# HorizonRobotics/GeoFlowSlam

Hardware: AMD Instinct MI355X
Metric: front-end frames/sec (ORB+match+GICP) on 640x480 RGBD (higher is better)
Workload: dtype u8/int32 (ORB, match) + f64 (GICP); 1 GPU; BASELINE.json configs[1]: 640x480 RGBD frame pair, ORB extract (1000 feats, 8 levels) + BF Hamming match + GMS filter + GICP on ~19k-pt clouds (stride-4 depth grid); batch_pairs_per_gpu=512, lanes_per_gpu=4, passes=K passes per lane chain, joined once, distinct_scenes_per_gpu=512, scene_seeds=1000..1511 (rank 0), global_batch_pairs=512, parallelism=frames sharded x1, no collective

## Files before the change

geoflowslam_amd/csrc/gicp.hip:

```cpp
#include <algorithm>
#include <atomic>
#include <cmath>
#include <cstdlib>
#include <memory>
#include <type_traits>

#include "gfs_common.hpp"
#include "glibc_math.hpp"
#include "voxel_qsort.hpp"
#include "wave_reduce.hpp"

namespace {

typedef unsigned long long u64;
constexpr u64 kInvalidKey = ~0ull;
constexpr int kCoordBits = 21;
constexpr int kCoordOffset = 1 << (kCoordBits - 1);
constexpr int kCoordMask = (1 << kCoordBits) - 1;
#ifndef GFS_FINE_BITS
#define GFS_FINE_BITS 6
#endif
constexpr int kFineBits = GFS_FINE_BITS, kFine = 1 << kFineBits;
static_assert(kFineBits >= 1 && kFineBits <= 6, "the x field of a cell sort key: 19 bits of cell + the sub-cell bits in 25");
constexpr int kCkSy = 25, kCkSz = 45;
constexpr int kCkOffX = 1 << 24, kCkOffY = 1 << 19, kCkOffZ = 1 << 18;
constexpr int kRed = 29;
constexpr int kLinBlock = 256;

struct PairState {
  double T[12];
  double newT[12];
  double delta[6];
  double H[21], b[6], e;
  double lambda;
  int outer, inner;
  int phase;
  int converged;
  int iterations;
  int inliers;
  int n_lin, n_err;
  int buf;
  int pad_;
};

struct GicpParams {
  double inv_leaf, cell, inv_cell, max_dist_sq, rot_eps, trans_eps;
  int max_iterations, k_neighbors;
  unsigned* tile_stats;
  int lin_tile;
  int nn_rings;
  int src_slot, only;
  int knn_exact;
};

__device__ __forceinline__ int fast_floor_d(double v) {
  const int n = (int)v;
  return n - (v < (double)n ? 1 : 0);
}
__device__ __forceinline__ u64 pack_key(int cx, int cy, int cz) {
  return (u64)(cx & kCoordMask) | ((u64)(cy & kCoordMask) << kCoordBits) | ((u64)(cz & kCoordMask) << (2 * kCoordBits));
}

__global__ __launch_bounds__(256) void k_voxel_keys(const float4* __restrict__ tgt, const float4* __restrict__ src,
                                                    const int* __restrict__ nt, const int* __restrict__ ns,
                                                    int stride_pts, int P, double inv_leaf, double max_vox, u64* __restrict__ keys,
                                                    unsigned* __restrict__ idx, int* __restrict__ counts, int only,
                                                    int* __restrict__ n_done4, int* __restrict__ n_heap, int* __restrict__ n_active4) {
  const int c = blockIdx.y, pair = c >> 1, which = c & 1;
  if (blockIdx.x == 0 && threadIdx.x < 4) {
    if (threadIdx.x == 0) n_heap[c] = 0;
    if (c == 0) {
      n_done4[threadIdx.x] = 0;
      n_active4[threadIdx.x] = 0;
    }
  }
  if (only >= 0 && which != only) return;
  const int n = min(which ? ns[pair] : nt[pair], P);
  const float4* in = (which ? src : tgt) + (size_t)pair * stride_pts;
  const int i = blockIdx.x * 256 + threadIdx.x;
  if (i == 0) counts[c] = n;
  if (i >= n) return;
  const float4 p = in[i];
  const double x = (double)p.x * inv_leaf, y = (double)p.y * inv_leaf, z = (double)p.z * inv_leaf;
  u64 key = kInvalidKey;
  if (fabs(x) < max_vox && fabs(y) < max_vox && fabs(z) < max_vox) {
    const int cx = fast_floor_d(x) + kCoordOffset, cy = fast_floor_d(y) + kCoordOffset, cz = fast_floor_d(z) + kCoordOffset;
// ... 987 lines not shown
    atomicAdd(util + slot, (unsigned)__popcll(m));
    atomicAdd(util + slot + 1, 1u);
  }
}
#define GFS_KNN_UTIL_STEP(util, slot) knn_util_step(util, slot)
#else
#define GFS_KNN_UTIL_STEP(util, slot)
#endif
__device__ __forceinline__ void knn_walk_own_row(const double4* __restrict__ p, const double4& q, int i, int lo, int hi, double slack,
                                                 int want, TopKey11& loc, unsigned* util = nullptr) {
  int r = i, l = i - 1;
  bool ra = r < hi, la = l >= lo;
  const int kw_at = max(want - 1, 0);
  while (ra || la) {
    GFS_KNN_UTIL_STEP(util, 0);
    const int j0 = min(r, hi - 1), j1 = max(l, lo), j2 = min(r + 1, hi - 1), j3 = max(l - 1, lo);
    const bool on2 = ra && r + 1 < hi, on3 = la && l - 1 >= lo;
    const double4 t0 = ld_pt(p, j0), t1 = ld_pt(p, j1), t2 = ld_pt(p, j2), t3 = ld_pt(p, j3);
    loc.push4(knn_key(t0, q, j0, ra), knn_key(t1, q, j1, la), knn_key(t2, q, j2, on2), knn_key(t3, q, j3, on3));
    const double kw = loc.at(kw_at);
    const double B = kw < TopKey11::kNone ? TopKey11::upper(kw) : TopKey11::kNone;
    if (ra) {
      r += 2;
      const double g = t2.x - slack - q.x;
      ra = r < hi && !(g > 0.0 && g * g > B);
    }
    if (la) {
      l -= 2;
      const double g = q.x - t3.x - slack;
      la = l >= lo && !(g > 0.0 && g * g > B);
    }
  }
}
__device__ __forceinline__ void knn_scan_runs4_keys(const double4* __restrict__ p, const double4& q, int b0, int l0, int b1, int l1,
                                                    int b2, int l2, int b3, int l3, TopKey11& loc, unsigned* util = nullptr) {
  const int c1 = l0, c2 = c1 + l1, c3 = c2 + l2, total = c3 + l3;
  const int o0 = b0, o1 = b1 - c1, o2 = b2 - c2, o3 = b3 - c3;
  for (int v = 0; v < total; v += 4) {
    GFS_KNN_UTIL_STEP(util, 2);
    int j[4];
#pragma unroll
    for (int u = 0; u < 4; u++) {
      const int vv = min(v + u, total - 1);
      j[u] = vv + (vv < c1 ? o0 : vv < c2 ? o1 : vv < c3 ? o2 : o3);
    }
    const int j0 = j[0], j1 = j[1], j2 = j[2], j3 = j[3];
    const double4 t0 = ld_pt(p, j0), t1 = ld_pt(p, j1), t2 = ld_pt(p, j2), t3 = ld_pt(p, j3);
    loc.push4(knn_key(t0, q, j0, true), knn_key(t1, q, j1, v + 1 < total), knn_key(t2, q, j2, v + 2 < total),
              knn_key(t3, q, j3, v + 3 < total));
  }
}

__device__ __forceinline__ void knn_write_cov(const TopK<10>& best, int kk, const double4* __restrict__ p, double* __restrict__ out) {
  const int n = min(best.found, kk);
  if (n < 5) {
    out[0] = 1;
    out[1] = 0;
    out[2] = 0;
    out[3] = 1;
    out[4] = 0;
    out[5] = 1;
    return;
  }
  double sp[3] = {0, 0, 0}, sc[6] = {0, 0, 0, 0, 0, 0};
#pragma unroll
  for (int k = 0; k < 10; k++) {
    if (k < n) {
      const double4 t = p[best.id[k]];
      sp[0] += t.x;
      sp[1] += t.y;
      sp[2] += t.z;
      sc[0] += t.x * t.x;
      sc[1] += t.x * t.y;
      sc[2] += t.x * t.z;
      sc[3] += t.y * t.y;
      sc[4] += t.y * t.z;
      sc[5] += t.z * t.z;
    }
  }
  const double dn = (double)n;
  const double mean[3] = {sp[0] / dn, sp[1] / dn, sp[2] / dn};
  double cv[6];
  cv[0] = (sc[0] - mean[0] * sp[0]) / dn;
  cv[1] = (sc[1] - mean[1] * sp[0]) / dn;
// ... 37 lines not shown
}

__device__ __forceinline__ void knn_scan_runs4(const double4* __restrict__ p, const double4& q, int b0, int l0, int b1, int l1, int b2,
                                               int l2, int b3, int l3, TopK<10>& loc) {
  const int c1 = l0, c2 = c1 + l1, c3 = c2 + l2, total = c3 + l3;
  const int o0 = b0, o1 = b1 - c1, o2 = b2 - c2, o3 = b3 - c3;
  for (int v = 0; v < total; v += 4) {
    int j[4];
#pragma unroll
    for (int u = 0; u < 4; u++) {
      const int vv = min(v + u, total - 1);
      j[u] = vv + (vv < c1 ? o0 : vv < c2 ? o1 : vv < c3 ? o2 : o3);
    }
    const double4 t0 = p[j[0]], t1 = p[j[1]], t2 = p[j[2]], t3 = p[j[3]];
    {
      const double ddx = t0.x - q.x, ddy = t0.y - q.y, ddz = t0.z - q.z;
      loc.push(j[0], ddx * ddx + ddy * ddy + ddz * ddz);
    }
    if (v + 1 < total) {
      const double ddx = t1.x - q.x, ddy = t1.y - q.y, ddz = t1.z - q.z;
      loc.push(j[1], ddx * ddx + ddy * ddy + ddz * ddz);
    }
    if (v + 2 < total) {
      const double ddx = t2.x - q.x, ddy = t2.y - q.y, ddz = t2.z - q.z;
      loc.push(j[2], ddx * ddx + ddy * ddy + ddz * ddz);
    }
    if (v + 3 < total) {
      const double ddx = t3.x - q.x, ddy = t3.y - q.y, ddz = t3.z - q.z;
      loc.push(j[3], ddx * ddx + ddy * ddy + ddz * ddz);
    }
  }
}

__global__ __launch_bounds__(128) void k_knn_cov(const double4* __restrict__ pts, const u64* __restrict__ ucell,
                                                 const unsigned* __restrict__ ubegin, const int* __restrict__ n_ucell,
                                                 const int* __restrict__ m_counts, const int* __restrict__ bbox,
                                                 const unsigned* __restrict__ grid, const int* __restrict__ ginfo,
                                                 int* __restrict__ ginfo_rw, unsigned* __restrict__ hard_list,
                                                 double* __restrict__ hard_d, int nchunks, int npairs, int P, GicpParams prm,
                                                 double* __restrict__ cov6) {
  int pair, which, chunk;
  if (!xcd_pair_map(nchunks, npairs, 2, &pair, &which, &chunk)) return;
  if (prm.only >= 0 && which != prm.only) return;
  const int c = 2 * pair + which;
  const int m = m_counts[c];
  const int i = chunk * 128 + threadIdx.x;
  if (i >= m) return;
  const unsigned* G = grid + (size_t)c * (kGridCap + 1);
  const int* gi = ginfo + 8 * c;
  const double4* p = pts + (size_t)c * P;
  const u64* uc = ucell + (size_t)c * (P + 1);
  const unsigned* ub = ubegin + (size_t)c * (P + 1);
  const int nu = n_ucell[c];
  const double4 q = p[i];
  const int cx = fast_floor_d(q.x * prm.inv_cell) + kCoordOffset, cy = fast_floor_d(q.y * prm.inv_cell) + kCoordOffset,
            cz = fast_floor_d(q.z * prm.inv_cell) + kCoordOffset;
  TopKey11 best;
  const int kk = min(prm.k_neighbors, 10);
  const int want = min(kk, m);
  bool certified = false;
  double kth_for_deferred = TopKey11::kNone;
  {
    best.init();
    const double cell2 = prm.cell * prm.cell;
    const double ux = q.x * prm.inv_cell - (double)(cx - kCoordOffset), uy = q.y * prm.inv_cell - (double)(cy - kCoordOffset),
                 uz = q.z * prm.inv_cell - (double)(cz - kCoordOffset);
    const double lx0 = fmax(ux - 1e-9, 0.0) * prm.cell, lx2 = fmax(1.0 - ux - 1e-9, 0.0) * prm.cell;
    const double ly[3] = {fmax(uy - 1e-9, 0.0) * prm.cell, 0.0, fmax(1.0 - uy - 1e-9, 0.0) * prm.cell};
    const double lz[3] = {fmax(uz - 1e-9, 0.0) * prm.cell, 0.0, fmax(1.0 - uz - 1e-9, 0.0) * prm.cell};
    {
      int j0, j1;
      row_range(gi, G, uc, ub, nu, cx - 1, cx + 1, cy, cz, &j0, &j1);
#ifdef GFS_KNN_OWN_ROW_SCAN
      knn_scan_run_keys(p, q, j0, j1, best);
#else
      if (i >= j0 && i < j1)
        knn_walk_own_row(p, q, i, j0, j1, prm.cell * (1.0 / kFine + 1e-9), want, best, prm.tile_stats);
      else
        knn_scan_run_keys(p, q, j0, j1, best);
#endif
    }
    auto kth_bound = [&]() {
      const double kw = best.at(max(want - 1, 0));
      return kw < TopKey11::kNone ? TopKey11::upper(kw) : TopKey11::kNone;
    };
    constexpr int rows[2][4] = {{1, 3, 5, 7}, {0, 2, 6, 8}};
#pragma unroll
    for (int round = 0; round < 2; round++) {
      const double B = kth_bound();
      int rb[4], rl[4];
#pragma unroll
      for (int u = 0; u < 4; u++) {
        const int t9 = rows[round][u], dy = t9 % 3, dz = t9 / 3;
        const double row2 = ly[dy] * ly[dy] + lz[dz] * lz[dz];
        rb[u] = 0;
        rl[u] = 0;
        if (row2 <= B) {
          int e[4];
          row_cells3(gi, G, uc, ub, nu, cx, cy + dy - 1, cz + dz - 1, e);
          const int b0 = row2 + lx0 * lx0 <= B ? e[0] : e[1], e0 = row2 + lx2 * lx2 <= B ? e[3] : e[2];
          rb[u] = b0;
          rl[u] = e0 - b0;
        }
      }
      knn_scan_runs4_keys(p, q, rb[0], rl[0], rb[1], rl[1], rb[2], rl[2], rb[3], rl[3], best, prm.tile_stats);
    }
#ifdef GFS_KNN_UTIL
    if (prm.tile_stats) {
      GFS_KNN_UTIL_STEP(prm.tile_stats, 4);
      int j0, j1;
      row_range(gi, G, uc, ub, nu, cx - 1, cx + 1, cy, cz, &j0, &j1);
      atomicAdd(prm.tile_stats + 6, (unsigned)(j1 - j0));
    }
#endif
    const double fx = fmin(ux + 1.0, 2.0 - ux), fy = fmin(uy + 1.0, 2.0 - uy), fz = fmin(uz + 1.0, 2.0 - uz);
    const double reach = fmax(fmin(fx, fmin(fy, fz)) - 1e-9, 1.0) * prm.cell;
    const double kw = best.at(max(want - 1, 0)), kn = best.at(want);
    certified = want > 0 && kw < TopKey11::kNone && TopKey11::upper(kw) <= fmax(reach * reach, cell2) &&
                !(kn < TopKey11::kNone && TopKey11::same_high_bits(kw, kn));
    certified = (certified || want == 0) && !prm.knn_exact;
    kth_for_deferred = kw < TopKey11::kNone ? TopKey11::upper(kw) : TopKey11::kNone;
  }
  if (!certified) {
    const int slot = atomicAdd(&ginfo_rw[8 * c + 7], 1);
    hard_list[(size_t)c * P + slot] = (unsigned)i;
    hard_d[(size_t)c * P + slot] = kth_for_deferred;
    return;
  }
  TopK<10> res;
  res.found = 0;
#pragma unroll
  for (int k = 0; k < 10; k++) {
    res.id[k] = best.k[k] < TopKey11::kNone ? TopKey11::index(best.k[k]) : -1;
    res.found += best.k[k] < TopKey11::kNone ? 1 : 0;
  }
  knn_write_cov(res, kk, p, cov6 + ((size_t)c * P + i) * 6);
}

// ... 545 lines not shown
      atomicAdd(src.util + 7, 1u);
    }
  }
#endif
  row(cy, cz, 0.0);
  unsigned need = 0;
#pragma unroll
  for (int t8 = 0; t8 < 8; t8++) {
    const int t9 = t8 < 4 ? t8 : t8 + 1, dy = t9 % 3, dz = t9 / 3;
    const double a = dy == 0 ? ly0 : dy == 2 ? ly2 : 0.0, c = dz == 0 ? lz0 : dz == 2 ? lz2 : 0.0;
    if (a * a + c * c <= B) need |= 1u << t8;
  }
  while (__any(need != 0)) {
#ifdef GFS_LIN_UTIL
    if (src.util) {
      const unsigned long long m = __ballot(need != 0);
      if ((int)(threadIdx.x & 63) == __ffsll((long long)__ballot(1)) - 1) {
        atomicAdd(src.util + 2, (unsigned)__popcll(m));
        atomicAdd(src.util + 3, 1u);
      }
    }
#endif
    if (need != 0) {
      const int t8 = __ffs(need) - 1;
      need &= need - 1;
      const int t9 = t8 < 4 ? t8 : t8 + 1, dy = t9 % 3, dz = t9 / 3;
      const double a = dy == 0 ? ly0 : dy == 2 ? ly2 : 0.0, c = dz == 0 ? lz0 : dz == 2 ? lz2 : 0.0;
      const double row2 = a * a + c * c;
      if (row2 <= B) row(cy + dy - 1, cz + dz - 1, row2);
    }
  }
}

__device__ __forceinline__ int lin_stage_tile(LinTile& T, bool inrange, int cx, int cy, int cz, const double4* __restrict__ tp,
                                              const int* __restrict__ gi, const unsigned* __restrict__ G) {
  const int tid = threadIdx.x, lane = tid & 63, wave = tid >> 6;
  if (!gi[6]) return 1;
  if (tid < 4) T.box[tid] = (tid & 1) ? INT_MIN : INT_MAX;
  if (tid < kTileRows) {
    T.row_a[tid] = INT_MAX;
    T.row_b[tid] = INT_MIN;
  }
  __syncthreads();
  {
    int v[4] = {inrange ? cy : INT_MAX, inrange ? -cy : INT_MAX, inrange ? cz : INT_MAX, inrange ? -cz : INT_MAX};
#pragma unroll
    for (int ofs = 32; ofs > 0; ofs >>= 1)
#pragma unroll
      for (int k = 0; k < 4; k++) v[k] = min(v[k], __shfl_xor(v[k], ofs, 64));
    if (lane == 0 && v[0] != INT_MAX) {
      atomicMin(&T.box[0], v[0]);
      atomicMax(&T.box[1], -v[1]);
      atomicMin(&T.box[2], v[2]);
      atomicMax(&T.box[3], -v[3]);
    }
  }
  __syncthreads();
  const int cymin = T.box[0], cymax = T.box[1], czmin = T.box[2], czmax = T.box[3];
  if (cymin > cymax) return 2;
  const long long nyl = (long long)cymax - cymin + 3, nzl = (long long)czmax - czmin + 3;
  if (nyl * nzl > kTileRows) return 3;
  const int ny = (int)nyl, nz = (int)nzl, nrows = ny * nz, y0 = cymin - 1, z0 = czmin - 1;
  if (inrange) {
    const int r = (cy - y0) + ny * (cz - z0);
    atomicMin(&T.row_a[r], cx);
    atomicMax(&T.row_b[r], cx);
// ... 189 lines not shown
  v[3] = fmsub2(F.Q[5], F.px, F.Q[3], F.pz);
  v[4] = fmsub2(F.Q[8], F.px, F.Q[6], F.pz);
  v[5] = fmsub2(F.Q[6], F.py, F.Q[7], F.px);
  v[6] = fmsub2(F.u[1], F.pz, F.u[2], F.py);
  v[7] = fmsub2(F.u[2], F.px, F.u[0], F.pz);
  v[8] = fmsub2(F.u[0], F.py, F.u[1], F.px);
  v[9] = -F.u[0];
  v[10] = -F.u[1];
  v[11] = -F.u[2];
  v[12] = 0.5 * fma3(F.w[0], F.u[0], F.w[1], F.u[1], F.w[2], F.u[2]);
  v[13] = 1.0;
}
__device__ __forceinline__ void lin_factor_batch_a(const LinFactor& F, double (&v)[15]) {
#pragma unroll
  for (int k = 0; k < 15; k++) v[k] = 0;
  if (!F.on) return;
#pragma unroll
  for (int c = 0; c < 3; c++)
#pragma unroll
    for (int r = 0; r < 3; r++) v[3 * c + r] = -F.Q[c + 3 * r];
#pragma unroll
  for (int k = 0; k < 6; k++) v[9 + k] = F.N[k];
}
__device__ __forceinline__ void lin_factor_accumulate(const LinFactor& F, double (&acc)[kRed]) {
  double a[15], b[14];
  lin_factor_batch_a(F, a);
  lin_factor_batch_b(F, b);
#pragma unroll
  for (int k = 0; k < 15; k++) acc[kLinMapA[k]] += a[k];
#pragma unroll
  for (int k = 0; k < 14; k++) acc[kLinMapB[k]] += b[k];
}

template <class Src>
__device__ __forceinline__ void gicp_lin_point(const Src& src, int i, const double4 p, double tx, double ty, double tz, int cx, int cy, int cz,
                                               bool in_range, const double* __restrict__ T12, bool has_prev, int prev_j, const double4 prev_q,
                                               int pair, int cs, int ct, int P,
                                               const double4* __restrict__ pts, const double* __restrict__ cov6,
                                               const u64* __restrict__ ucell, const unsigned* __restrict__ ubegin,
                                               const int* __restrict__ n_ucell, const unsigned* __restrict__ G,
                                               const int* __restrict__ gi, const GicpParams& prm, int* __restrict__ tgt_index,
                                               double* __restrict__ maha6, LinFactor& F) {
  {
    const double4* tp = pts + (size_t)ct * P;
    const u64* uc = ucell + (size_t)ct * (P + 1);
    const unsigned* ub = ubegin + (size_t)ct * (P + 1);
    const int nu = n_ucell[ct];
    double best = 1.79769313486231570e308;
    int bj = -1;
    if (in_range) {
      if (prm.nn_rings <= 1) {
        if (has_prev && prev_j >= 0) {
          best = (prev_q.x - tx) * (prev_q.x - tx) + (prev_q.y - ty) * (prev_q.y - ty) + (prev_q.z - tz) * (prev_q.z - tz);
          bj = prev_j;
        }
        nn_search27(src, prm, tx, ty, tz, cx, cy, cz, best, bj);
      } else {
      {
        int j0s[9], j1s[9];
#pragma unroll
        for (int t9 = 0; t9 < 9; t9++)
          row_range(gi, G, uc, ub, nu, cx - 1, cx + 1, cy + (t9 % 3) - 1, cz + t9 / 3 - 1, &j0s[t9], &j1s[t9]);
#pragma unroll
        for (int t9 = 0; t9 < 9; t9++) {
          const int jb = j0s[t9], je = j1s[t9];
          for (int j = jb; j < je; j += 4) {
            const int ja = min(j + 1, je - 1), jb2 = min(j + 2, je - 1), jc = min(j + 3, je - 1);
            const double4 q0 = tp[j], q1 = tp[ja], q2 = tp[jb2], q3 = tp[jc];
            const double d0 = (q0.x - tx) * (q0.x - tx) + (q0.y - ty) * (q0.y - ty) + (q0.z - tz) * (q0.z - tz);
            const double d1 = (q1.x - tx) * (q1.x - tx) + (q1.y - ty) * (q1.y - ty) + (q1.z - tz) * (q1.z - tz);
            const double d2 = (q2.x - tx) * (q2.x - tx) + (q2.y - ty) * (q2.y - ty) + (q2.z - tz) * (q2.z - tz);
            const double d3 = (q3.x - tx) * (q3.x - tx) + (q3.y - ty) * (q3.y - ty) + (q3.z - tz) * (q3.z - tz);
            if (d0 < best) { best = d0; bj = j; }
            if (d1 < best) { best = d1; bj = ja; }
            if (d2 < best) { best = d2; bj = jb2; }
            if (d3 < best) { best = d3; bj = jc; }
          }
        }
      }
      const bool done1 = (bj >= 0 && best <= prm.cell * prm.cell) || prm.nn_rings <= 1;
      for (int r = 2; !done1 && r <= prm.nn_rings; r++) {
        best = 1.79769313486231570e308;
        bj = -1;
        for (int dz = -r; dz <= r; dz++)
          for (int dy = -r; dy <= r; dy++) {
            int j0, j1;
            row_range(gi, G, uc, ub, nu, cx - r, cx + r, cy + dy, cz + dz, &j0, &j1);
            for (int j = j0; j < j1; j++) {
              const double4 q = tp[j];
// ... 19 lines not shown

__device__ __forceinline__ void lin_image(const double4& p, const double* __restrict__ T12, const GicpParams& prm, double& tx, double& ty,
                                          double& tz, int& cx, int& cy, int& cz, bool& in_range) {
  const double* R = T12;
  const double* t = T12 + 9;
  tx = R[0] * p.x + R[3] * p.y + R[6] * p.z + t[0];
  ty = R[1] * p.x + R[4] * p.y + R[7] * p.z + t[1];
  tz = R[2] * p.x + R[5] * p.y + R[8] * p.z + t[2];
  cx = fast_floor_d(tx * prm.inv_cell) + kCoordOffset;
  cy = fast_floor_d(ty * prm.inv_cell) + kCoordOffset;
  cz = fast_floor_d(tz * prm.inv_cell) + kCoordOffset;
  in_range = fabs(tx) < 2.0e4 && fabs(ty) < 2.0e4 && fabs(tz) < 2.0e4;
}

#ifdef GFS_LIN_WAVES
#define GFS_LIN_OCC __attribute__((amdgpu_waves_per_eu(GFS_LIN_WAVES, 8)))
#else
#define GFS_LIN_OCC __attribute__((amdgpu_waves_per_eu(5, 8)))
#endif
struct CoopSync {
  unsigned arrive;
  unsigned gen;
};
__device__ void pair_step_last(PairState* S, const double* part, const double* epart, int nblk_pair, int phase, double rot_eps,
                               double trans_eps, int max_iterations, int pair, int* n_done, int* act_next, int* n_act_next, double* s_part,
                               double* s_sum);

__device__ __forceinline__ double gicp_trial_error(const double4 q, double tx, double ty, double tz, const double* __restrict__ M) {
  const double r0 = q.x - tx, r1 = q.y - ty, r2 = q.z - tz;
  const double m0 = M[0] * r0 + M[1] * r1 + M[2] * r2, m1 = M[1] * r0 + M[3] * r1 + M[4] * r2, m2 = M[2] * r0 + M[4] * r1 + M[5] * r2;
  return 0.5 * (r0 * m0 + r1 * m1 + r2 * m2);
}

template <bool kTiled, bool kFuse>
__global__ __launch_bounds__(kLinBlock) GFS_LIN_OCC void k_gicp_linearize(PairState* __restrict__ st,
                                                              const double4* __restrict__ pts,
                                                              const double* __restrict__ cov6, const u64* __restrict__ ucell,
                                                              const unsigned* __restrict__ ubegin,
                                                              const int* __restrict__ n_ucell, const int* __restrict__ m_counts,
                                                              const unsigned* __restrict__ grid, const int* __restrict__ ginfo,
                                                              int nchunks, int npairs, int P, GicpParams prm,
                                                              int* __restrict__ tgt_index, double* __restrict__ maha6, size_t buf_stride,
                                                              double* __restrict__ partial, double* __restrict__ epartial, int nblk,
                                                              const int* __restrict__ act, const int* __restrict__ n_act,
                                                              CoopSync* __restrict__ sync, int* __restrict__ n_done,
                                                              int* __restrict__ act_next, int* __restrict__ n_act_next,
                                                              int* __restrict__ n_act_clear) {
  __shared__ typename std::conditional<kTiled, LinTile, int>::type tile;
  if constexpr (kFuse) {
    if (blockIdx.x == 0 && threadIdx.x == 0) *n_act_clear = 0;
  }
  int pair, sub, chunk;
  if (act) {
    const int slot = blockIdx.x / nchunks;
    if (slot >= *n_act) return;
    pair = act[slot];
    chunk = blockIdx.x - slot * nchunks;
  } else if (!xcd_pair_map(nchunks, npairs, 1, &pair, &sub, &chunk)) {
    return;
  }
  const int cs = 2 * pair + prm.src_slot, ct = 2 * pair + 1 - prm.src_slot;
  const PairState* Sp = st + pair;
  const int phase = Sp->phase, n_lin = Sp->n_lin, cur = Sp->buf;
  const double* Tp = phase == 0 ? Sp->T : Sp->newT;
  double T12[12];
#pragma unroll
  for (int k = 0; k < 12; k++) T12[k] = Tp[k];
// ... 8 lines not shown
  const double* maha_cur = maha6 + (size_t)cur * buf_stride * 6;
  const int prev_j = ti_cur[(size_t)pair * P + i];
  const int nblk_pair = (ms + kLinBlock - 1) / kLinBlock;
  if (phase == 2 || chunk >= (kFuse ? max(nblk_pair, 1) : nblk_pair)) return;
  const bool has_prev = n_lin > 0;
  double4 prev_q = make_double4(0, 0, 0, 0);
  if (has_prev && i < ms && prev_j >= 0) prev_q = tp[prev_j];
  LinFactor F;
  F.on = false;
  double tx = 0, ty = 0, tz = 0;
  int cx = 0, cy = 0, cz = 0;
  bool in_range = false;
  if (i < ms) lin_image(p, T12, prm, tx, ty, tz, cx, cy, cz, in_range);
  if (phase != 0) {
    double e[1] = {0.0};
    if (i < ms && prev_j >= 0) e[0] = gicp_trial_error(prev_q, tx, ty, tz, maha_cur + ((size_t)pair * P + i) * 6);
    wave_reduce_store<1, kFuse>(e, epartial + ((size_t)pair * nblk + chunk) * kLinWaves, wave_slot);
  }
  if (phase != 3) {
    const int wr = phase == 0 ? cur : cur ^ 1;
    int* ti_wr = tgt_index + (size_t)wr * buf_stride;
    double* maha_wr = maha6 + (size_t)wr * buf_stride * 6;
    bool tiled = false;
    if constexpr (kTiled) {
      const int why = prm.nn_rings <= 1 ? lin_stage_tile(tile, i < ms && in_range, cx, cy, cz, tp, gi, G) : 6;
      tiled = why == 0;
      if (prm.tile_stats && threadIdx.x == 0) atomicAdd(prm.tile_stats + why, 1u);
    }
    if (i < ms) {
      bool done = false;
      if constexpr (kTiled) {
        if (tiled) {
          const NnTile src{&tile, tile.box[0] - 1, tile.box[2] - 1, tile.box[1] - tile.box[0] + 3};
          gicp_lin_point(src, i, p, tx, ty, tz, cx, cy, cz, in_range, T12, has_prev, prev_j, prev_q, pair, cs, ct, P, pts, cov6, ucell, ubegin,
                         n_ucell, G, gi, prm, ti_wr, maha_wr, F);
          done = true;
        }
      }
      if (!done) {
#ifdef GFS_LIN_UTIL
        const NnGlobal src{tp, gi, G, ucell + (size_t)ct * (P + 1), ubegin + (size_t)ct * (P + 1), n_ucell[ct], prm.tile_stats};
#else
        const NnGlobal src{tp, gi, G, ucell + (size_t)ct * (P + 1), ubegin + (size_t)ct * (P + 1), n_ucell[ct]};
#endif
        gicp_lin_point(src, i, p, tx, ty, tz, cx, cy, cz, in_range, T12, has_prev, prev_j, prev_q, pair, cs, ct, P, pts, cov6, ucell, ubegin, n_ucell,
                       G, gi, prm, ti_wr, maha_wr, F);
      }
    }
    double* dst = partial + ((size_t)pair * nblk + chunk) * kLinWaves * kRed;
    {
      double vb[14];
      lin_factor_batch_b(F, vb);
      wave_reduce_store_map<14, kFuse>(vb, kLinMapB, dst, wave_slot);
    }
    {
      double va[15];
      lin_factor_batch_a(F, va);
      wave_reduce_store_map<15, kFuse>(va, kLinMapA, dst, wave_slot);
    }
  }
  if constexpr (kFuse) {
    __shared__ double s_part[8 * 32], s_sum[32];
    __shared__ int s_last;
    asm volatile("s_waitcnt vmcnt(0)" ::: "memory");
    __syncthreads();
    if (threadIdx.x == 0) {
      const unsigned old = __hip_atomic_fetch_add(&sync[pair].arrive, 1u, __ATOMIC_RELAXED, __HIP_MEMORY_SCOPE_AGENT);
      s_last = old + 1 == (unsigned)max(nblk_pair, 1) ? 1 : 0;
    }
    __syncthreads();
    if (s_last) {
      pair_step_last(st + pair, partial + (size_t)pair * nblk * kLinWaves * kRed, epartial + (size_t)pair * nblk * kLinWaves, nblk_pair, phase,
                     prm.rot_eps, prm.trans_eps, prm.max_iterations, pair, n_done, act_next, n_act_next, s_part, s_sum);
      if (threadIdx.x == 0) st_ag(&sync[pair].arrive, 0u);
    }
  }
}

__device__ void solve_and_propose(const double* H21, const double* b6, double lambda, const double* T12, double* delta6,
// ... 848 lines not shown
static int gicp_run(gfs_gicp* h, const void* dev_target, const void* dev_nt, const void* dev_source, const void* dev_ns, int B,
                    int stride_pts, const double* init_T, const gfs_gicp_config* cfg, gfs_gicp_result* out, void* stream,
                    bool streaming) {
  GFS_REQUIRE(h && (streaming || (dev_target && dev_nt)) && dev_source && dev_ns && B > 0 && stride_pts > 0 && cfg && out,
              GFS_ERR_INVALID_ARG, "gfs_gicp_align: invalid argument");
  GFS_REQUIRE(B <= h->Bmax, GFS_ERR_CAPACITY, "batch %d exceeds handle max_batch %d", B, h->Bmax);
  GFS_REQUIRE(cfg->downsampling_resolution > 0 && cfg->max_correspondence_distance > 0 && cfg->num_neighbors >= 1 &&
                  cfg->num_neighbors <= 10,
              GFS_ERR_UNSUPPORTED, "gfs_gicp: need resolution > 0, max_corr > 0, 1 <= num_neighbors <= 10");
  std::lock_guard<std::recursive_mutex> lk(h->mu);
  GFS_HIP(hipSetDevice(h->device));
  hipStream_t s = stream ? (hipStream_t)stream : h->stream;
  const int P = h->P, C2 = 2 * B;
  const bool optimistic_sort = h->lm_rounds && !h->sort_all_kernels && h->sort_all_hold == 0;
  if (h->sort_all_hold > 0 && !h->sort_all_kernels) h->sort_all_hold--;
  GicpParams prm;
  prm.inv_leaf = 1.0 / cfg->downsampling_resolution;
  prm.cell = cfg->max_correspondence_distance;
  if (const char* e = getenv("GFS_GICP_CELL")) prm.cell = atof(e);
  prm.inv_cell = 1.0 / prm.cell;
  prm.nn_rings = (int)std::ceil(cfg->max_correspondence_distance / prm.cell - 1e-12);
  if (prm.nn_rings < 1) prm.nn_rings = 1;
  prm.lin_tile = 0;
  prm.tile_stats = h->tile_stats_on ? h->d_tile_stats.p : nullptr;
  if (const char* e = getenv("GFS_GICP_LIN_TILE")) prm.lin_tile = atoi(e) != 0;
  prm.max_dist_sq = cfg->max_correspondence_distance * cfg->max_correspondence_distance;
  prm.rot_eps = cfg->rotation_eps;
  prm.trans_eps = cfg->translation_eps;
  prm.max_iterations = cfg->max_iterations;
  prm.k_neighbors = cfg->num_neighbors;
  prm.src_slot = 1;
  prm.only = -1;
  prm.knn_exact = getenv("GFS_GICP_KNN_EXACT") && atoi(getenv("GFS_GICP_KNN_EXACT")) != 0;
  if (streaming) {
    GFS_REQUIRE(h->last_B == B && h->last_leaf == cfg->downsampling_resolution && h->last_cell == prm.cell &&
                    h->last_k == cfg->num_neighbors,
                GFS_ERR_INVALID_ARG,
                "gfs_gicp_align_next: needs a previous call on this handle with the same batch size and preprocessing "
                "parameters (its source clouds are this call's targets)");
    prm.src_slot = 1 - h->last_src_slot;
    prm.only = prm.src_slot;
  }
  const float4* in_even = (const float4*)(streaming ? (prm.src_slot == 0 ? dev_source : nullptr) : dev_target);
  const float4* in_odd = (const float4*)(streaming ? (prm.src_slot == 1 ? dev_source : nullptr) : dev_source);
  const int* n_even = (const int*)(streaming ? (prm.src_slot == 0 ? dev_ns : (const void*)h->d_zero.p) : dev_nt);
  const int* n_odd = (const int*)(streaming ? (prm.src_slot == 1 ? dev_ns : (const void*)h->d_zero.p) : dev_ns);
  for (int b = 0; b < B; b++)
    for (int k = 0; k < 16; k++) h->h_initT.p[16 * b + k] = init_T ? init_T[16 * b + k] : (k % 5 == 0 ? 1.0 : 0.0);
  const int npts = std::min(stride_pts, P);
  const double max_vox = std::min(1.0e6, (double)((1 << 18) - 2) * prm.cell * prm.inv_leaf);
  GFS_LAUNCH("k_voxel_keys", k_voxel_keys, dim3(gfs::div_up(npts, 256), C2), dim3(256), 0, s, in_even, in_odd, n_even, n_odd,
             stride_pts, P, prm.inv_leaf, max_vox, h->d_keys0.p, h->d_val0.p, h->d_counts.p, prm.only, h->d_ndone.p, h->d_nheap.p,
             h->d_nactive.p);
  if (h->stable_voxel_order) {
    GFS_LAUNCH("k_radix_sort", k_radix_sort, dim3(C2), dim3(1024), 0, s, h->d_keys0.p, h->d_keys1.p, h->d_val0.p, h->d_val1.p,
               h->d_counts.p, P, h->d_which.p, h->d_kinfo1.p, prm.only, kCoordBits, 2 * kCoordBits);
  } else {
    const int leaf_parts = std::max(1, std::min(64, P / 1024));
    int rc_leaf = 0;
    GFS_HIP(voxel_qsort_top(h, C2, s, prm.only, optimistic_sort ? h->d_ndone.p + 1 : nullptr));
    static const bool exact_ties = getenv("GFS_GICP_VOXEL_TIES") && strcmp(getenv("GFS_GICP_VOXEL_TIES"), "exact") == 0;
    const bool narrow_only = optimistic_sort && h->vqs_lds && P <= 1024 * kVqsLdsGvE;
    rc_leaf = exact_ties ? voxel_qsort_leaves(h, C2, leaf_parts, s, prm.only, narrow_only)
                         : voxel_qsort_leaves(h, C2, leaf_parts, s, prm.only, narrow_only, in_even, in_odd, stride_pts);
    if (rc_leaf) return rc_leaf;
  }
  const int tiles = P / 1024, wg_parts = std::max(1, std::min(std::min(8, tiles), 384 / std::max(1, prm.only >= 0 ? C2 / 2 : C2)));
  const int tiles_per_part = gfs::div_up(tiles, wg_parts);
  GFS_LAUNCH("k_voxel_reduce", k_voxel_reduce, dim3(C2, wg_parts), dim3(1024), 0, s, in_even, in_odd, stride_pts, h->d_keys0.p,
             h->d_keys1.p, h->d_val0.p, h->d_val1.p, h->d_which.p, h->d_counts.p, P, prm.inv_cell, h->d_tmp.p, h->d_ck0.p, h->d_ci0.p,
             h->d_m.p, prm.only, tiles_per_part, h->d_bbox.p);
  if (optimistic_sort && h->vqs_lds && P <= 1024 * kCsE) {
    GFS_LAUNCH("k_cell_sort_lds", k_cell_sort_lds, dim3(C2), dim3(1024), kCsLdsBytes, s, h->d_ck0.p, h->d_ci0.p, h->d_m.p, P,
               h->d_which2.p, h->d_kinfo2.p, prm.only, h->d_ndone.p + 1);
  } else {
    GFS_LAUNCH("k_radix_sort", k_radix_sort, dim3(C2), dim3(1024), 0, s, h->d_ck0.p, h->d_ck1.p, h->d_ci0.p, h->d_ci1.p,
               h->d_m.p, P, h->d_which2.p, h->d_kinfo2.p, prm.only, kCkSy, kCkSz);
  }
  GFS_LAUNCH("k_cell_build", k_cell_build, dim3(C2, wg_parts), dim3(1024), 0, s, h->d_tmp.p, h->d_ck0.p, h->d_ck1.p, h->d_ci0.p,
             h->d_ci1.p, h->d_which2.p, h->d_m.p, P, h->d_pts.p, h->d_ucell.p, h->d_ubegin.p, h->d_nucell.p, h->d_bbox.p, h->d_kinfo2.p,
             prm.only);
  GFS_LAUNCH("k_grid_fill", k_grid_fill, dim3(kGridFillParts, C2), dim3(256), 0, s, h->d_ucell.p, h->d_ubegin.p, h->d_nucell.p, h->d_m.p,
             h->d_bbox.p, P, h->d_grid.p, h->d_ginfo.p, h->d_far2.p, prm.only);
  const int knn_chunks = gfs::div_up(npts, 128);
  GFS_LAUNCH("k_knn_cov", k_knn_cov, dim3(xcd_grid(knn_chunks, B, 2)), dim3(128), 0, s, h->d_pts.p, h->d_ucell.p,
             h->d_ubegin.p, h->d_nucell.p, h->d_m.p, h->d_bbox.p, h->d_grid.p, h->d_ginfo.p, h->d_ginfo.p, h->d_hard.p,
             h->d_hard_d.p, knn_chunks, B, P, prm, h->d_cov6.p);
  const int far_chunks = std::max(1, std::min(32, knn_chunks));
  GFS_LAUNCH("k_knn_cov_far", (k_knn_cov_far<16, 2, true>), dim3(xcd_grid(far_chunks, B, 2)), dim3(256), 0, s, h->d_pts.p,
             h->d_ucell.p, h->d_ubegin.p, h->d_nucell.p, h->d_m.p, h->d_bbox.p, h->d_grid.p, h->d_ginfo.p, h->d_hard.p,
             h->d_hard_d.p, h->d_far2.p, far_chunks, B, P, prm, h->d_cov6.p);
  const int far2_chunks = std::max(1, std::min(32, knn_chunks));
  static const bool far2_groups = getenv("GFS_GICP_FAR2") && strcmp(getenv("GFS_GICP_FAR2"), "groups") == 0;
  if (far2_groups)
    GFS_LAUNCH("k_knn_cov_far_groups", (k_knn_cov_far<64, 4, false>), dim3(xcd_grid(4, B, 2)), dim3(256), 0, s, h->d_pts.p,
               h->d_ucell.p, h->d_ubegin.p, h->d_nucell.p, h->d_m.p, h->d_bbox.p, h->d_grid.p, h->d_ginfo.p, h->d_hard.p,
               h->d_hard_d.p, h->d_far2.p, 4, B, P, prm, h->d_cov6.p);
  else
    GFS_LAUNCH("k_knn_cov_far_wg", k_knn_cov_far_wg, dim3(xcd_grid(far2_chunks, B, 2)), dim3(256), 0, s, h->d_pts.p, h->d_ucell.p,
               h->d_ubegin.p, h->d_nucell.p, h->d_m.p, h->d_bbox.p, h->d_grid.p, h->d_ginfo.p, h->d_hard.p, h->d_hard_d.p,
               h->d_far2.p, far2_chunks, B, P, prm, h->d_cov6.p);
  GFS_LAUNCH("k_gicp_init", k_gicp_init, dim3(gfs::div_up(B, 64)), dim3(64), 0, s, h->d_state.p, h->hd_initT, B,
             prm.max_iterations, h->d_ndone.p, h->d_sync.p);
  if (!h->lm_rounds) {
    GFS_LAUNCH("k_gicp_lm", k_gicp_lm, dim3(B), dim3(kLmBlock), 0, s, h->d_state.p, h->d_pts.p, h->d_cov6.p, h->d_ucell.p,
               h->d_ubegin.p, h->d_nucell.p, h->d_m.p, h->d_grid.p, h->d_ginfo.p, B, P, prm, h->d_tgt_index.p, h->d_maha6.p);
  } else {
    const int nblk_run = gfs::div_up(npts, kLinBlock);
    const int max_rounds = std::max(1, prm.max_iterations) * 11 + 2;
    const size_t buf_stride = (size_t)h->Bmax * P;
    int known_done = 0;
    static const bool lin_wg_default = !getenv("GFS_GICP_LIN_WG") || atoi(getenv("GFS_GICP_LIN_WG")) / 64 * 64 >= 256;
    const bool coop_ok = h->coop && !h->coop_failed && !prm.lin_tile && lin_wg_default && h->coop_cap > 0 && prm.max_iterations > 0;
    const int coop_budget = h->coop_cap / 2;
    auto launch_coop = [&](int n_ub, const int* act_list, const int* n_act_list) -> bool {
      static const int max_wg = getenv("GFS_GICP_COOP_MAXWG") ? std::max(1, atoi(getenv("GFS_GICP_COOP_MAXWG"))) : (1 << 30);
      const int want = std::min(std::min(n_ub * nblk_run, coop_budget), std::max(n_ub, max_wg));
      const int got = CoopBudget::reserve(h->device, want, std::max(n_ub, want / 2), coop_budget);
      if (got <= 0) return false;
      h->coop_reserved += got;
      h->coop_launches++;
      h->coop_last_wgs = got;
      GFS_LAUNCH("k_gicp_lm_coop", k_gicp_lm_coop, dim3(got), dim3(kLinBlock), 0, s, h->d_state.p, h->d_pts.p, h->d_cov6.p, h->d_ucell.p,
                 h->d_ubegin.p, h->d_nucell.p, h->d_m.p, h->d_grid.p, h->d_ginfo.p, nblk_run, P, prm, h->d_tgt_index.p, h->d_maha6.p,
                 buf_stride, h->d_partial.p, h->d_epartial.p, h->nblk, act_list, n_act_list, n_ub, h->d_sync.p, h->d_ndone.p, h->d_ndone.p + 2);
      return true;
    };
    bool in_coop = coop_ok && (long long)B * nblk_run <= coop_budget && launch_coop(B, nullptr, nullptr);
    for (int round = 0; round < max_rounds && !in_coop; round++) {
      const int ub = B - known_done;
      if (coop_ok && round >= 2 && ub < B && (double)ub * nblk_run <= h->coop_tail * coop_budget &&
          launch_coop(ub, h->d_active.p + (size_t)(round % 3) * B, h->d_nactive.p + (round % 3))) {
        in_coop = true;
        break;
      }
      const bool listed = round >= 2 && 4 * ub <= B;
      const int* act = listed ? h->d_active.p + (size_t)(round % 3) * B : nullptr;
      const int* n_act = h->d_nactive.p + (round % 3);
      int* act_next = h->d_active.p + (size_t)((round + 1) % 3) * B;
      int* n_act_next = h->d_nactive.p + ((round + 1) % 3);
      int* n_act_clear = h->d_nactive.p + ((round + 2) % 3);
      const dim3 grid_pts(listed ? std::max(ub, 1) * nblk_run : xcd_grid(nblk_run, B, 1));
      static const int lin_wg = getenv("GFS_GICP_LIN_WG") ? std::max(64, std::min(256, atoi(getenv("GFS_GICP_LIN_WG")) / 64 * 64)) : 256;
      const int per = kLinBlock / (lin_wg == 128 ? 128 : lin_wg == 256 ? 256 : 64), wg = kLinBlock / per;
      const dim3 grid_w(listed ? std::max(ub, 1) * nblk_run * per : xcd_grid(nblk_run * per, B, 1));
      const bool fuse = h->fuse_step && wg == kLinBlock;
      if (prm.lin_tile) {
        GFS_LAUNCH("k_gicp_linearize", (k_gicp_linearize<true, false>), grid_pts, dim3(kLinBlock), 0, s, h->d_state.p,
                   h->d_pts.p, h->d_cov6.p, h->d_ucell.p, h->d_ubegin.p, h->d_nucell.p, h->d_m.p, h->d_grid.p, h->d_ginfo.p,
                   nblk_run, B, P, prm, h->d_tgt_index.p, h->d_maha6.p, buf_stride, h->d_partial.p, h->d_epartial.p, h->nblk, act, n_act,
                   nullptr, nullptr, nullptr, nullptr, nullptr);
      } else if (fuse) {
        GFS_LAUNCH("k_gicp_linearize", (k_gicp_linearize<false, true>), grid_w, dim3(wg), 0, s, h->d_state.p,
                   h->d_pts.p, h->d_cov6.p, h->d_ucell.p, h->d_ubegin.p, h->d_nucell.p, h->d_m.p, h->d_grid.p, h->d_ginfo.p,
                   nblk_run * per, B, P, prm, h->d_tgt_index.p, h->d_maha6.p, buf_stride, h->d_partial.p, h->d_epartial.p, h->nblk, act, n_act,
                   h->d_sync.p, h->d_ndone.p, act_next, n_act_next, n_act_clear);
      } else {
        GFS_LAUNCH("k_gicp_linearize", (k_gicp_linearize<false, false>), grid_w, dim3(wg), 0, s, h->d_state.p,
                   h->d_pts.p, h->d_cov6.p, h->d_ucell.p, h->d_ubegin.p, h->d_nucell.p, h->d_m.p, h->d_grid.p, h->d_ginfo.p,
                   nblk_run * per, B, P, prm, h->d_tgt_index.p, h->d_maha6.p, buf_stride, h->d_partial.p, h->d_epartial.p, h->nblk, act, n_act,
                   nullptr, nullptr, nullptr, nullptr, nullptr);
      }
      if (!fuse || prm.lin_tile)
        GFS_LAUNCH("k_gicp_step", k_gicp_step, dim3(B), dim3(256), 0, s, h->d_state.p, h->d_partial.p, h->d_epartial.p, h->d_m.p, h->nblk, prm,
                   h->d_ndone.p, act_next, n_act_next, n_act_clear);
      const int nslot = h->ahead + 1, slot = round % nslot;
      GFS_HIP(hipMemcpyAsync(h->h_ndone.p + 2 * slot, h->d_ndone.p, 2 * sizeof(int), hipMemcpyDeviceToHost, s));
      GFS_HIP(hipEventRecord(h->ev_round[slot], s));
      if (round >= h->ahead) {
        const int pslot = (round - h->ahead) % nslot;
        GFS_HIP(hipEventSynchronize(h->ev_round[pslot]));
        if (optimistic_sort && h->h_ndone.p[2 * pslot + 1] > 0) {
          GFS_HIP(hipStreamSynchronize(s));
          h->sort_all_kernels = true;
          const int rc_again = gicp_run(h, dev_target, dev_nt, dev_source, dev_ns, B, stride_pts, init_T, cfg, out, stream, streaming);
          h->sort_all_kernels = false;
          h->sort_all_hold = 64;
          return rc_again;
        }
        known_done = h->h_ndone.p[2 * pslot];
        if (known_done >= B) break;
      }
    }
  }
  int* const last_look = h->h_ndone.p + 2 * (gfs_gicp::kAheadMax + 1);
  last_look[0] = last_look[1] = last_look[2] = 0;
  GFS_LAUNCH("k_gicp_publish", k_gicp_publish, dim3(std::max(1, std::min(16, gfs::div_up(B * kStateWords, 256)))), dim3(256), 0, s, h->d_state.p,
             h->d_m.p, h->d_ndone.p, B, reinterpret_cast<u64*>(h->hd_state), h->hd_m, h->hd_last);
  const hipError_t rc_sync = hipStreamSynchronize(s);
  CoopBudget::release(h->device, h->coop_reserved);
  h->coop_reserved = 0;
// ... 213 lines not shown
```

Baseline: 42030 frames/s.

## Add wave-coherent fused neighbor walks for KNN and GICP NN search

Adds alternative neighbor-search loops that merge the own-row and neighbor-row scans into one wave-uniform loop, so lanes that finish early pick up the next row instead of idling at divergence points. These are selectable by environment variable for both the covariance KNN and the GICP linearize nearest-neighbor search. It also adds an occupancy hint to the KNN kernel. The defaults keep the round-based walk, and the fused NN mode disables the cooperative launch path.

```diff
diff --git a/geoflowslam_amd/csrc/gicp.hip b/geoflowslam_amd/csrc/gicp.hip
--- a/geoflowslam_amd/csrc/gicp.hip
+++ b/geoflowslam_amd/csrc/gicp.hip
@@ -51,7 +51,9 @@
   int nn_rings;
   int src_slot, only;
   int knn_exact;
+  int nn_rounds, knn_rounds;
 };
+constexpr int kNnWalkRounds = 1, kKnnWalkRounds = 1;
 
 __device__ __forceinline__ int fast_floor_d(double v) {
   const int n = (int)v;
@@ -1105,11 +1107,13 @@
     }
   }
 }
-__device__ __forceinline__ void knn_scan_runs4_keys(const double4* __restrict__ p, const double4& q, int b0, int l0, int b1, int l1,
-                                                    int b2, int l2, int b3, int l3, TopKey11& loc, unsigned* util = nullptr) {
-  const int c1 = l0, c2 = c1 + l1, c3 = c2 + l2, total = c3 + l3;
-  const int o0 = b0, o1 = b1 - c1, o2 = b2 - c2, o3 = b3 - c3;
-  for (int v = 0; v < total; v += 4) {
+struct KnnRuns4 {
+  int c1, c2, c3, total, o0, o1, o2, o3;
+  __device__ __forceinline__ void set(int b0, int l0, int b1, int l1, int b2, int l2, int b3, int l3) {
+    c1 = l0, c2 = c1 + l1, c3 = c2 + l2, total = c3 + l3;
+    o0 = b0, o1 = b1 - c1, o2 = b2 - c2, o3 = b3 - c3;
+  }
+  __device__ __forceinline__ void step4(const double4* __restrict__ p, const double4& q, int v, TopKey11& loc, unsigned* util) const {
     GFS_KNN_UTIL_STEP(util, 2);
     int j[4];
 #pragma unroll
@@ -1122,7 +1126,7 @@
     loc.push4(knn_key(t0, q, j0, true), knn_key(t1, q, j1, v + 1 < total), knn_key(t2, q, j2, v + 2 < total),
               knn_key(t3, q, j3, v + 3 < total));
   }
-}
+};
 
 __device__ __forceinline__ void knn_write_cov(const TopK<10>& best, int kk, const double4* __restrict__ p, double* __restrict__ out) {
   const int n = min(best.found, kk);
@@ -1226,7 +1230,8 @@
   }
 }
 
-__global__ __launch_bounds__(128) void k_knn_cov(const double4* __restrict__ pts, const u64* __restrict__ ucell,
+template <bool kRounds>
+__global__ __launch_bounds__(128) __attribute__((amdgpu_waves_per_eu(4, 8))) void k_knn_cov(const double4* __restrict__ pts, const u64* __restrict__ ucell,
                                                  const unsigned* __restrict__ ubegin, const int* __restrict__ n_ucell,
                                                  const int* __restrict__ m_counts, const int* __restrict__ bbox,
                                                  const unsigned* __restrict__ grid, const int* __restrict__ ginfo,
@@ -1278,26 +1283,53 @@
       const double kw = best.at(max(want - 1, 0));
       return kw < TopKey11::kNone ? TopKey11::upper(kw) : TopKey11::kNone;
     };
-    constexpr int rows[2][4] = {{1, 3, 5, 7}, {0, 2, 6, 8}};
-#pragma unroll
-    for (int round = 0; round < 2; round++) {
+    KnnRuns4 runs;
+    auto rows4 = [&](auto round_c, auto in_loop) {
+      constexpr int rows[2][4] = {{1, 3, 5, 7}, {0, 2, 6, 8}};
       const double B = kth_bound();
+      int xc = cx, yc = cy, zc = cz;
+      double ly0 = ly[0], ly2 = ly[2], lz0 = lz[0], lz2 = lz[2], lxa = lx0, lxb = lx2;
+      if constexpr (decltype(in_loop)::value)
+        asm volatile("" : "+v"(xc), "+v"(yc), "+v"(zc), "+v"(ly0), "+v"(ly2), "+v"(lz0), "+v"(lz2), "+v"(lxa), "+v"(lxb));
+      const double lyc[3] = {ly0, 0.0, ly2}, lzc[3] = {lz0, 0.0, lz2};
       int rb[4], rl[4];
 #pragma unroll
       for (int u = 0; u < 4; u++) {
+        constexpr int round = decltype(round_c)::value;
         const int t9 = rows[round][u], dy = t9 % 3, dz = t9 / 3;
-        const double row2 = ly[dy] * ly[dy] + lz[dz] * lz[dz];
+        const double row2 = lyc[dy] * lyc[dy] + lzc[dz] * lzc[dz];
         rb[u] = 0;
         rl[u] = 0;
         if (row2 <= B) {
           int e[4];
-          row_cells3(gi, G, uc, ub, nu, cx, cy + dy - 1, cz + dz - 1, e);
-          const int b0 = row2 + lx0 * lx0 <= B ? e[0] : e[1], e0 = row2 + lx2 * lx2 <= B ? e[3] : e[2];
+          row_cells3(gi, G, uc, ub, nu, xc, yc + dy - 1, zc + dz - 1, e);
+          const int b0 = row2 + lxa * lxa <= B ? e[0] : e[1], e0 = row2 + lxb * lxb <= B ? e[3] : e[2];
           rb[u] = b0;
           rl[u] = e0 - b0;
         }
       }
-      knn_scan_runs4_keys(p, q, rb[0], rl[0], rb[1], rl[1], rb[2], rl[2], rb[3], rl[3], best, prm.tile_stats);
+      runs.set(rb[0], rl[0], rb[1], rl[1], rb[2], rl[2], rb[3], rl[3]);
+    };
+    if constexpr (kRounds) {
+      rows4(std::integral_constant<int, 0>{}, std::false_type{});
+      for (int v = 0; v < runs.total; v += 4) runs.step4(p, q, v, best, prm.tile_stats);
+      rows4(std::integral_constant<int, 1>{}, std::false_type{});
+      for (int v = 0; v < runs.total; v += 4) runs.step4(p, q, v, best, prm.tile_stats);
+    } else {
+      rows4(std::integral_constant<int, 0>{}, std::false_type{});
+      int v = 0;
+      bool diag = true;
+      while (__any(v < runs.total || diag)) {
+        if (v >= runs.total && diag) {
+          diag = false;
+          rows4(std::integral_constant<int, 1>{}, std::true_type{});
+          v = 0;
+        }
+        if (v < runs.total) {
+          runs.step4(p, q, v, best, prm.tile_stats);
+          v += 4;
+        }
+      }
     }
 #ifdef GFS_KNN_UTIL
     if (prm.tile_stats) {
@@ -1909,6 +1941,117 @@
   }
 }
 
+template <class Src>
+__device__ __forceinline__ void nn_search27_fused(const Src& src, const GicpParams& prm, double tx, double ty, double tz, int cx, int cy,
+                                                  int cz, double& best, int& bj) {
+  double B = fmin(prm.max_dist_sq, best);
+  const double ux = tx * prm.inv_cell - (double)(cx - kCoordOffset), uy = ty * prm.inv_cell - (double)(cy - kCoordOffset),
+               uz = tz * prm.inv_cell - (double)(cz - kCoordOffset);
+  const double ly0 = fmax(uy - 1e-9, 0.0) * prm.cell, ly2 = fmax(1.0 - uy - 1e-9, 0.0) * prm.cell;
+  const double lz0 = fmax(uz - 1e-9, 0.0) * prm.cell, lz2 = fmax(1.0 - uz - 1e-9, 0.0) * prm.cell;
+  const double slack = prm.cell * (1.0 / kFine + 1e-9);
+  auto row2_of = [&](int t8, int& dy, int& dz) {
+    const int t9 = t8 < 4 ? t8 : t8 + 1;
+    dy = t9 % 3;
+    dz = t9 / 3;
+    const double a = dy == 0 ? ly0 : dy == 2 ? ly2 : 0.0, c = dz == 0 ? lz0 : dz == 2 ? lz2 : 0.0;
+    return a * a + c * c;
+  };
+  int lo, hi, d, r, l;
+  bool ra, la;
+  auto enter = [&](int y, int z) {
+    int e[4];
+    d = src.cells3(cx, y, z, e);
+    lo = e[0];
+    hi = e[3];
+    const int n1 = e[2] - e[1];
+    r = e[1] + min(max((int)(ux * (double)n1), 0), n1);
+    l = r - 1;
+    ra = hi > lo && r < hi;
+    la = hi > lo && l >= lo;
+  };
+#ifdef GFS_LIN_UTIL
+  if (src.util) {
+    const unsigned long long m = __ballot(1);
+    if ((int)(threadIdx.x & 63) == __ffsll((long long)m) - 1) {
+      atomicAdd(src.util + 6, (unsigned)__popcll(m));
+      atomicAdd(src.util + 7, 1u);
+    }
+  }
+#endif
+  constexpr unsigned kOwnRow = 1u << 8;
+  double row2 = 0.0;
+  unsigned need = kOwnRow;
+  enter(cy, cz);
+  while (__any(ra || la || need != 0)) {
+    if (!(ra || la) && need != 0) {
+      if (need == kOwnRow) {
+        need = 0;
+#pragma unroll
+        for (int t8 = 0; t8 < 8; t8++) {
+          int dy, dz;
+          if (row2_of(t8, dy, dz) <= B) need |= 1u << t8;
+        }
+      }
+#ifdef GFS_LIN_UTIL
+      if (src.util) {
+        const unsigned long long m = __ballot(need != 0);
+        if ((int)(threadIdx.x & 63) == __ffsll((long long)__ballot(1)) - 1) {
+          atomicAdd(src.util + 2, (unsigned)__popcll(m));
+          atomicAdd(src.util + 3, 1u);
+        }
+      }
+#endif
+      if (need != 0) {
+        const int t8 = __ffs(need) - 1;
+        need &= need - 1;
+        int dy, dz;
+        const double r2 = row2_of(t8, dy, dz);
+        if (r2 <= B) {
+          row2 = r2;
+          enter(cy + dy - 1, cz + dz - 1);
+        }
+      }
+    }
+    if (ra || la) {
+#ifdef GFS_LIN_UTIL
+      if (src.util) {
+        const unsigned long long m = __ballot(1);
+        if ((int)(threadIdx.x & 63) == __ffsll((long long)m) - 1) {
+          atomicAdd(src.util + 4, (unsigned)__popcll(m));
+          atomicAdd(src.util + 5, 1u);
+        }
+      }
+#endif
+      const int j[4] = {min(r, hi - 1), max(l, lo), min(r + 1, hi - 1), max(l - 1, lo)};
+      double qx[4], dd[4];
+#pragma unroll
+      for (int u = 0; u < 4; u++) {
+        double qy, qz;
+        src.load(j[u] + d, qx[u], qy, qz);
+        dd[u] = (qx[u] - tx) * (qx[u] - tx) + (qy - ty) * (qy - ty) + (qz - tz) * (qz - tz);
+      }
+#pragma unroll
+      for (int u = 0; u < 4; u++)
+        if (dd[u] < best) {
+          best = dd[u];
+          bj = j[u];
+        }
+      B = fmin(prm.max_dist_sq, best);
+      if (ra) {
+        r += 2;
+        const double g = qx[2] - slack - tx;
+        ra = r < hi && !(g > 0.0 && g * g + row2 > B);
+      }
+      if (la) {
+        l -= 2;
+        const double g = tx - qx[3] - slack;
+        la = l >= lo && !(g > 0.0 && g * g + row2 > B);
+      }
+    }
+  }
+}
+
 __device__ __forceinline__ int lin_stage_tile(LinTile& T, bool inrange, int cx, int cy, int cz, const double4* __restrict__ tp,
                                               const int* __restrict__ gi, const unsigned* __restrict__ G) {
   const int tid = threadIdx.x, lane = tid & 63, wave = tid >> 6;
@@ -2164,7 +2307,7 @@
   for (int k = 0; k < 14; k++) acc[kLinMapB[k]] += b[k];
 }
 
-template <class Src>
+template <bool kFusedWalk = false, class Src>
 __device__ __forceinline__ void gicp_lin_point(const Src& src, int i, const double4 p, double tx, double ty, double tz, int cx, int cy, int cz,
                                                bool in_range, const double* __restrict__ T12, bool has_prev, int prev_j, const double4 prev_q,
                                                int pair, int cs, int ct, int P,
@@ -2186,7 +2329,8 @@
           best = (prev_q.x - tx) * (prev_q.x - tx) + (prev_q.y - ty) * (prev_q.y - ty) + (prev_q.z - tz) * (prev_q.z - tz);
           bj = prev_j;
         }
-        nn_search27(src, prm, tx, ty, tz, cx, cy, cz, best, bj);
+        if constexpr (kFusedWalk) nn_search27_fused(src, prm, tx, ty, tz, cx, cy, cz, best, bj);
+        else nn_search27(src, prm, tx, ty, tz, cx, cy, cz, best, bj);
       } else {
       {
         int j0s[9], j1s[9];
@@ -2272,7 +2416,7 @@
   return 0.5 * (r0 * m0 + r1 * m1 + r2 * m2);
 }
 
-template <bool kTiled, bool kFuse>
+template <bool kTiled, bool kFuse, bool kFusedWalk>
 __global__ __launch_bounds__(kLinBlock) GFS_LIN_OCC void k_gicp_linearize(PairState* __restrict__ st,
                                                               const double4* __restrict__ pts,
                                                               const double* __restrict__ cov6, const u64* __restrict__ ucell,
@@ -2347,8 +2491,8 @@
       if constexpr (kTiled) {
         if (tiled) {
           const NnTile src{&tile, tile.box[0] - 1, tile.box[2] - 1, tile.box[1] - tile.box[0] + 3};
-          gicp_lin_point(src, i, p, tx, ty, tz, cx, cy, cz, in_range, T12, has_prev, prev_j, prev_q, pair, cs, ct, P, pts, cov6, ucell, ubegin,
-                         n_ucell, G, gi, prm, ti_wr, maha_wr, F);
+          gicp_lin_point<kFusedWalk>(src, i, p, tx, ty, tz, cx, cy, cz, in_range, T12, has_prev, prev_j, prev_q, pair, cs, ct, P, pts, cov6,
+                                     ucell, ubegin, n_ucell, G, gi, prm, ti_wr, maha_wr, F);
           done = true;
         }
       }
@@ -2358,8 +2502,8 @@
 #else
         const NnGlobal src{tp, gi, G, ucell + (size_t)ct * (P + 1), ubegin + (size_t)ct * (P + 1), n_ucell[ct]};
 #endif
-        gicp_lin_point(src, i, p, tx, ty, tz, cx, cy, cz, in_range, T12, has_prev, prev_j, prev_q, pair, cs, ct, P, pts, cov6, ucell, ubegin, n_ucell,
-                       G, gi, prm, ti_wr, maha_wr, F);
+        gicp_lin_point<kFusedWalk>(src, i, p, tx, ty, tz, cx, cy, cz, in_range, T12, has_prev, prev_j, prev_q, pair, cs, ct, P, pts, cov6, ucell,
+                                   ubegin, n_ucell, G, gi, prm, ti_wr, maha_wr, F);
       }
     }
     double* dst = partial + ((size_t)pair * nblk + chunk) * kLinWaves * kRed;
@@ -3274,6 +3418,12 @@
   prm.src_slot = 1;
   prm.only = -1;
   prm.knn_exact = getenv("GFS_GICP_KNN_EXACT") && atoi(getenv("GFS_GICP_KNN_EXACT")) != 0;
+  auto walk_rounds = [](const char* name, int dflt) {
+    const char* e = getenv(name);
+    return !e ? dflt : !strcmp(e, "rounds") ? 1 : !strcmp(e, "fused") ? 0 : dflt;
+  };
+  prm.nn_rounds = walk_rounds("GFS_GICP_NN_WALK", kNnWalkRounds);
+  prm.knn_rounds = walk_rounds("GFS_GICP_KNN_WALK", kKnnWalkRounds);
   if (streaming) {
     GFS_REQUIRE(h->last_B == B && h->last_leaf == cfg->downsampling_resolution && h->last_cell == prm.cell &&
                     h->last_k == cfg->num_neighbors,
@@ -3325,9 +3475,9 @@
   GFS_LAUNCH("k_grid_fill", k_grid_fill, dim3(kGridFillParts, C2), dim3(256), 0, s, h->d_ucell.p, h->d_ubegin.p, h->d_nucell.p, h->d_m.p,
              h->d_bbox.p, P, h->d_grid.p, h->d_ginfo.p, h->d_far2.p, prm.only);
   const int knn_chunks = gfs::div_up(npts, 128);
-  GFS_LAUNCH("k_knn_cov", k_knn_cov, dim3(xcd_grid(knn_chunks, B, 2)), dim3(128), 0, s, h->d_pts.p, h->d_ucell.p,
-             h->d_ubegin.p, h->d_nucell.p, h->d_m.p, h->d_bbox.p, h->d_grid.p, h->d_ginfo.p, h->d_ginfo.p, h->d_hard.p,
-             h->d_hard_d.p, knn_chunks, B, P, prm, h->d_cov6.p);
+  GFS_LAUNCH("k_knn_cov", (prm.knn_rounds ? k_knn_cov<true> : k_knn_cov<false>), dim3(xcd_grid(knn_chunks, B, 2)), dim3(128), 0, s,
+             h->d_pts.p, h->d_ucell.p, h->d_ubegin.p, h->d_nucell.p, h->d_m.p, h->d_bbox.p, h->d_grid.p, h->d_ginfo.p, h->d_ginfo.p,
+             h->d_hard.p, h->d_hard_d.p, knn_chunks, B, P, prm, h->d_cov6.p);
   const int far_chunks = std::max(1, std::min(32, knn_chunks));
   GFS_LAUNCH("k_knn_cov_far", (k_knn_cov_far<16, 2, true>), dim3(xcd_grid(far_chunks, B, 2)), dim3(256), 0, s, h->d_pts.p,
              h->d_ucell.p, h->d_ubegin.p, h->d_nucell.p, h->d_m.p, h->d_bbox.p, h->d_grid.p, h->d_ginfo.p, h->d_hard.p,
@@ -3353,7 +3503,7 @@
     const size_t buf_stride = (size_t)h->Bmax * P;
     int known_done = 0;
     static const bool lin_wg_default = !getenv("GFS_GICP_LIN_WG") || atoi(getenv("GFS_GICP_LIN_WG")) / 64 * 64 >= 256;
-    const bool coop_ok = h->coop && !h->coop_failed && !prm.lin_tile && lin_wg_default && h->coop_cap > 0 && prm.max_iterations > 0;
+    const bool coop_ok = h->coop && !h->coop_failed && !prm.lin_tile && prm.nn_rounds && lin_wg_default && h->coop_cap > 0 && prm.max_iterations > 0;
     const int coop_budget = h->coop_cap / 2;
     auto launch_coop = [&](int n_ub, const int* act_list, const int* n_act_list) -> bool {
       static const int max_wg = getenv("GFS_GICP_COOP_MAXWG") ? std::max(1, atoi(getenv("GFS_GICP_COOP_MAXWG"))) : (1 << 30);
@@ -3388,17 +3538,20 @@
       const dim3 grid_w(listed ? std::max(ub, 1) * nblk_run * per : xcd_grid(nblk_run * per, B, 1));
       const bool fuse = h->fuse_step && wg == kLinBlock;
       if (prm.lin_tile) {
-        GFS_LAUNCH("k_gicp_linearize", (k_gicp_linearize<true, false>), grid_pts, dim3(kLinBlock), 0, s, h->d_state.p,
+        GFS_LAUNCH("k_gicp_linearize", (prm.nn_rounds ? k_gicp_linearize<true, false, false> : k_gicp_linearize<true, false, true>),
+                   grid_pts, dim3(kLinBlock), 0, s, h->d_state.p,
                    h->d_pts.p, h->d_cov6.p, h->d_ucell.p, h->d_ubegin.p, h->d_nucell.p, h->d_m.p, h->d_grid.p, h->d_ginfo.p,
                    nblk_run, B, P, prm, h->d_tgt_index.p, h->d_maha6.p, buf_stride, h->d_partial.p, h->d_epartial.p, h->nblk, act, n_act,
                    nullptr, nullptr, nullptr, nullptr, nullptr);
       } else if (fuse) {
-        GFS_LAUNCH("k_gicp_linearize", (k_gicp_linearize<false, true>), grid_w, dim3(wg), 0, s, h->d_state.p,
+        GFS_LAUNCH("k_gicp_linearize", (prm.nn_rounds ? k_gicp_linearize<false, true, false> : k_gicp_linearize<false, true, true>),
+                   grid_w, dim3(wg), 0, s, h->d_state.p,
                    h->d_pts.p, h->d_cov6.p, h->d_ucell.p, h->d_ubegin.p, h->d_nucell.p, h->d_m.p, h->d_grid.p, h->d_ginfo.p,
                    nblk_run * per, B, P, prm, h->d_tgt_index.p, h->d_maha6.p, buf_stride, h->d_partial.p, h->d_epartial.p, h->nblk, act, n_act,
                    h->d_sync.p, h->d_ndone.p, act_next, n_act_next, n_act_clear);
       } else {
-        GFS_LAUNCH("k_gicp_linearize", (k_gicp_linearize<false, false>), grid_w, dim3(wg), 0, s, h->d_state.p,
+        GFS_LAUNCH("k_gicp_linearize", (prm.nn_rounds ? k_gicp_linearize<false, false, false> : k_gicp_linearize<false, false, true>),
+                   grid_w, dim3(wg), 0, s, h->d_state.p,
                    h->d_pts.p, h->d_cov6.p, h->d_ucell.p, h->d_ubegin.p, h->d_nucell.p, h->d_m.p, h->d_grid.p, h->d_ginfo.p,
                    nblk_run * per, B, P, prm, h->d_tgt_index.p, h->d_maha6.p, buf_stride, h->d_partial.p, h->d_epartial.p, h->nblk, act, n_act,
                    nullptr, nullptr, nullptr, nullptr, nullptr);
```

Result: no change. 42000 frames/s (median of 2 runs) (-0.1%).
